# gabo99cas/minimal_volumetric_path_tracer

Hardware: AMD Instinct MI355X
Metric: Msamples/s (pixels×spp/s) at 1024²; per-channel RMSE vs CPU PPM (higher is better)
Workload: dtype f64; 1 GPU; ff 1024x1024x256spp default scene, sigma_a 0.001 sigma_s 0.009; width=1024, height=1024, spp=256, estimator=ff, parallelism=1 GPU, inflight=3

## Files before the change

minimal_volumetric_path_tracer_amd/_lib.py:

```python
from __future__ import annotations

import ctypes
import os
from ctypes import POINTER, c_char_p, c_double, c_int, c_int32, c_int64, c_uint64, c_void_p

import numpy as np

PKG_DIR = os.path.dirname(os.path.abspath(__file__))
LIB_PATH = os.environ.get("VPT_LIB") or os.path.join(PKG_DIR, "libvpt.so")
CLI_PATH = os.path.join(PKG_DIR, "vpt")

VPT_OK = 0
VPT_E_INVALID, VPT_E_TOO_MANY, VPT_E_NO_EMITTER, VPT_E_UNSUPPORTED, VPT_E_HIP, VPT_E_IO, VPT_E_INTERNAL = \
    -1, -2, -3, -4, -5, -6, -7
VPT_MAX_SPHERES = 64
FREE_FLIGHT, MIS_EQUIANGULAR, EXPLICIT_FREE, IMPLICIT_FREE, EXPLICIT_EQUIANGULAR, SURFACE_PT, RAY_MARCHING = 0, 1, 2, 3, 4, 5, 6
RAY_MARCHING_SA, RAY_MARCHING_GLOBAL, RAY_MARCHING_EXPLICIT = 7, 8, 9
HETERO_FREE = 10
HETERO_RATIO = 11
HETERO_EQUIANGULAR = 12
HETERO_MIS = 13
HETERO_CHROMATIC = 14
FB_F32, FB_F64 = 0, 1
GRID_NEAREST, GRID_TRILINEAR = 0, 1
# ... 138 lines not shown
                                        c_void_p, c_void_p, c_int, c_void_p, c_void_p, c_void_p, c_void_p, c_void_p, c_void_p,
                                        c_void_p, c_void_p, c_void_p]),
    ("vpt_grid_chroma_probe", c_int, [c_void_p, c_double, c_double, c_void_p, c_void_p, c_void_p, c_int, c_void_p, c_void_p,
                                      c_void_p, c_void_p, c_void_p, c_void_p]),
    ("vpt_grid_chroma_probe_host", c_int, [POINTER(vpt_grid_desc), c_void_p, c_int, c_int, c_void_p, c_void_p, c_void_p,
                                           c_void_p, c_void_p, c_int, c_void_p, c_void_p, c_void_p, c_void_p, c_void_p,
                                           c_void_p]),
    ("vpt_write_ppm", c_int, [c_char_p, c_void_p, c_int, c_int, c_int]),
    ("vpt_encode_ppm", c_int64, [c_void_p, c_int, c_int, c_int, c_void_p, c_int64]),
    ("vpt_last_error", c_char_p, []),
    ("vpt_abi_version", c_int, []),
    ("vpt_build_id", c_char_p, []),
]


def lib() -> ctypes.CDLL:
    global _lib
    if _lib is None:
        if not os.path.exists(LIB_PATH):
            raise RuntimeError(
                f"{LIB_PATH} is missing: build it with `python -c 'import __graft_entry__ as g; g.build()'` "
                "(or `make -C minimal_volumetric_path_tracer_amd/csrc`); there is no CPU fallback"
            )
        L = ctypes.CDLL(LIB_PATH)
        for name, res, args in PROTOTYPES:
            fn = getattr(L, name)
            fn.restype = res
            fn.argtypes = args
        _lib = L
    return _lib


def build_id() -> str:
    return lib().vpt_build_id().decode()


def check(rc: int) -> None:
    if rc != VPT_OK:
        msg = lib().vpt_last_error()
        raise VPTError(rc, msg.decode() if msg else "")
# ... 1 lines not shown
```

minimal_volumetric_path_tracer_amd/csrc/vpt_device.h:

```cpp
#ifndef VPT_DEVICE_H
#define VPT_DEVICE_H

#include <hip/hip_runtime.h>
#include <stdint.h>

#include <type_traits>

#include "vpt_math.h"
#include "vpt_rng.h"
#include "vpt_scene.h"

#define VPT_DEV __device__ static inline __attribute__((always_inline))
#define VPT_PI 3.14159265358979323846
#define VPT_MAXFLOAT ((double)3.40282346638528859812e+38F)
#define VPT_DBL_MAX 1.7976931348623157e+308
#ifndef VPT_ISECT_UNROLL
#define VPT_ISECT_UNROLL 5
#endif
#ifndef VPT_DECIDE_GROUP
#define VPT_DECIDE_GROUP 5
#endif
static_assert(VPT_DECIDE_GROUP >= 1, "spheres are taken G >= 1 at a time");

namespace vpt {

#define VPT_UNLIKELY(c) __builtin_expect(!!(c), 0)
#define VPT_LIKELY(c) __builtin_expect(!!(c), 1)

#define ISECT_SQRT(x) vm_sqrt(x)
#ifndef VPT_ISECT_CLASS
#define VPT_ISECT_CLASS 1
#endif

#ifndef VPT_SECTIONS
#define VPT_SECTIONS 0
#endif
enum {
    SECT_SCHED = 0, SECT_LOAD, SECT_S_PLIGHT, SECT_S_MIS, SECT_S_MIS_ISECT, SECT_S_BDSF, SECT_M_SS, SECT_M_SS_DIR,
    SECT_M_SS_ISECT, SECT_M_SS_SHADOW, SECT_M_PHASE, SECT_CONT, SECT_A_PREP, SECT_A_DECIDE, SECT_A_ISECT, SECT_STORE,
    SECT_S_TOTAL, SECT_M_TOTAL, SECT_A_CAMERA, SECT_A_DECIDE_IN, SECT_M_SHADOW_IN, SECT_A_CAMERA_IN, SECT_M_EQA,
    SECT_M_TR, SECT_A_UNIT, SECT_A_R2, SECT_A_PICK, SECT_A_LOG, SECT_A_CLASS, SECT_A_ALLFRESH, SECT_USED,
    SECT_N = 32
};
#if VPT_SECTIONS
static __device__ unsigned long long g_vpt_sect[3 * SECT_N];
__device__ static inline __attribute__((always_inline)) uint32_t* sect_lds()
{
    __shared__ uint32_t a[8][3 * SECT_USED];
    return &a[(threadIdx.x >> 6) & 7][0];
}
#endif
__device__ static inline __attribute__((always_inline)) uint32_t sect_now()
{
#if VPT_SECTIONS
    return (uint32_t)__builtin_amdgcn_s_memtime();
#else
// ... 3 lines not shown
__device__ static inline __attribute__((always_inline)) void sect_add(int k, uint32_t t0)
{
#if VPT_SECTIONS
    const uint32_t dt = sect_now() - t0;
    const unsigned long long act = (unsigned long long)__ballot(1);
    const int first = __ffsll(act) - 1;
    if ((int)(threadIdx.x & 63) == first) {
        uint32_t* a = sect_lds();
        a[k] += dt;
        a[SECT_USED + k] += 1;
        a[2 * SECT_USED + k] += (uint32_t)__popcll(act);
    }
#else
    (void)k;
    (void)t0;
#endif
}
__device__ static inline __attribute__((always_inline)) void sect_init()
{
#if VPT_SECTIONS
    for (int l = threadIdx.x & 63; l < 3 * SECT_USED; l += 64) sect_lds()[l] = 0;
#endif
}
__device__ static inline __attribute__((always_inline)) void sect_flush()
{
#if VPT_SECTIONS
    for (int l = threadIdx.x & 63; l < 3 * SECT_USED; l += 64) {
        const uint32_t v = sect_lds()[l];
        atomicAdd(&g_vpt_sect[l < SECT_USED ? l : l < 2 * SECT_USED ? SECT_N + l - SECT_USED : 2 * SECT_N + l - 2 * SECT_USED],
                  (unsigned long long)v);
// ... 144 lines not shown
        double cc = ocx * ocx + ocy * ocy + ocz * ocz;
        double det = b * b - cc + g.r2;
        sphere_test<ZR>(b, det, i, tmin, id, contact);
    }
    smp.tests(skip3 ? S->n_non3 : n);
    if (contact) {
        t = tmin;
        return 1;
    }
    t = 0;
    return 0;
}

template <int G, bool COUNT, bool ZR = false, class TAB = const double (*)[4]>
VPT_DEV int scene_intersect_grouped(const DevScene* __restrict__ S, Sampler<COUNT>& smp, dv3 o, dv3 d, double& t,
                                    int& id, bool cam = false, TAB cam_oc = nullptr)
{
    static_assert(G >= 1, "spheres are taken G >= 1 at a time");
    double tmin = VPT_DBL_MAX;
    contact_t contact = 0;
    const int n = S->n;
    int i = 0;
    for (; i + G <= n; i += G) {
        double b[G], det[G];
        if (cam) {
#pragma unroll
            for (int k = 0; k < G; ++k) {
                const double ocx = cam_oc[i + k][0], ocy = cam_oc[i + k][1], ocz = cam_oc[i + k][2], cc = cam_oc[i + k][3];
                b[k] = ocx * d.x + ocy * d.y + ocz * d.z;
                det[k] = b[k] * b[k] - cc + S->geo[i + k].r2;
            }
        } else {
#pragma unroll
            for (int k = 0; k < G; ++k) {
                const GeoSphere g = S->geo[i + k];
                const double ocx = o.x - g.px, ocy = o.y - g.py, ocz = o.z - g.pz;
                b[k] = ocx * d.x + ocy * d.y + ocz * d.z;
// ... 1171 lines not shown

template <bool COUNT>
VPT_DEV bool continue_path(Sampler<COUNT>& smp, const Path& p, const Medium& m)
{
    if (m.max_depth > 0 && p.depth >= m.max_depth) return false;
    if (COUNT) smp.cnt.iterations++;
    const double q = 1 - 0.6;
    return !(smp.next() < q);
}

template <int EST>
VPT_DEV constexpr bool est_free_flight() { return EST == 0 || EST == 2 || EST == 3; }

template <int EST, bool COUNT, bool HOIST = false, class TAB = const double (*)[4]>
VPT_DEV int decide(const DevScene* __restrict__ S, Sampler<COUNT>& smp, Path& p, Event& e, const Medium& m,
                   bool cam = false, TAB cam_oc = nullptr, uint64_t m_emitter = 0)
{
    constexpr bool hoist = HOIST && (EST == 0 || EST == 2);
    const double sigma_t = m.sigma_a + m.sigma_s;
    int id = 0;
    double t = 0.0;
    int h_count = 0, h_src = 0;
    double h_x = 0;
    gm_log_pair h_lp = {0, 0};
    if constexpr (hoist) {
        h_count = S->n_emit;
        if (VPT_LIKELY(h_count != 0)) {
            h_src = emit_pick(S, (int)(smp.next() * h_count), h_count);
            h_x = 1 - smp.next();
            h_lp = gm_log_pair_of(h_x);
        }
    }
    SECT_BEGIN(di);
#if VPT_DUP == DUP_DECIDE_ISECT
    {
        dv3 o2 = p.o, d2 = p.d;
        vpt_opaque(o2);
        vpt_opaque(d2);
        double t2 = 0;
        int id2 = 0;
        const int h2 = scene_intersect_grouped<VPT_DECIDE_GROUP>(S, smp, o2, d2, t2, id2);
        vpt_sink(t2);
        vpt_sink(id2);
        vpt_sink(h2);
    }
#endif
    const bool hit = scene_intersect_grouped<VPT_DECIDE_GROUP>(S, smp, p.o, p.d, t, id, cam, cam_oc);
    SECT_END(di, SECT_A_ISECT);
    if constexpr (EST == 5) {
        if (COUNT) smp.cnt.iterations++;
        e.t = t;
        e.id = id;
        e.src = 0;
        if (!hit) return EV_END;
        if (S->sph[id].radiance[0] > 0) {
            if (p.depth < 1) p.L = sph_rad(S, id);
            return EV_END;
        }
        return EV_SURF;
    }
    if (!hit) t = VPT_MAXFLOAT;
    e.t = t;
    e.id = id;
// ... 619 lines not shown
```

minimal_volumetric_path_tracer_amd/csrc/vpt_host.cpp:

```cpp
#include <math.h>
#include <stdarg.h>
#include <stdio.h>
#include <stdlib.h>
#include <string.h>

#include <string>
#include <vector>

#include <thread>

#include "vpt_accum.h"
#include "vpt_grid.h"
#include "vpt_grid_eqa.h"
#include "vpt_grid_mis.h"
#include "vpt_grid_chroma.h"
#include "vpt_internal.h"
#include "vpt_rng.h"

static thread_local std::string g_err;

int vpt_fail(int code, const char* fmt, ...)
{
    char buf[512];
    va_list ap;
    va_start(ap, fmt);
    vsnprintf(buf, sizeof buf, fmt, ap);
// ... 28 lines not shown
    }
    return VPT_OK;
}

void vpt_int_cam_table(const double* o, const double* centre, size_t stride, int n, double (*oc)[4])
{
    for (int i = 0; i < n; ++i, centre += stride) {
        const double ocx = o[0] - centre[0], ocy = o[1] - centre[1], ocz = o[2] - centre[2];
        oc[i][0] = ocx;
        oc[i][1] = ocy;
        oc[i][2] = ocz;
        oc[i][3] = ocx * ocx + ocy * ocy + ocz * ocz;
    }
}

extern "C" {

int vpt_debug_cam_table(const vpt_sphere* spheres, int n, const double* o, double* out)
{
    if (!spheres || !o || !out || n < 0 || n > VPT_MAX_SPHERES) return vpt_fail(VPT_E_INVALID, "vpt_debug_cam_table: bad arguments");
    vpt_int_cam_table(o, spheres[0].p, sizeof(vpt_sphere) / sizeof(double), n, (double (*)[4])out);
    return VPT_OK;
}

const char* vpt_last_error(void) { return g_err.c_str(); }
int vpt_abi_version(void) { return VPT_ABI_VERSION; }

uint64_t vpt_stream_state(uint64_t seed, uint64_t pixel_idx, uint64_t sample)
{
    return vpt_stream_start(seed, pixel_idx, sample);
}
// ... 444 lines not shown
```

minimal_volumetric_path_tracer_amd/csrc/vpt_internal.h:

```cpp
#ifndef VPT_INTERNAL_H
#define VPT_INTERNAL_H

#include <stddef.h>

#include "../../include/vpt.h"

int vpt_fail(int code, const char* fmt, ...);
void vpt_clear_error(void);

int vpt_int_device(const vpt_context* ctx);
const unsigned* vpt_int_guard_flag(const vpt_context* ctx);
int vpt_int_check_guard(vpt_context* ctx, const char* who);
int vpt_int_check_params(const vpt_context* ctx, const vpt_params* p);
int vpt_int_pool_pass(vpt_context* ctx, const vpt_params* p, int C, int k0, int k1, const unsigned* d_tiles,
                      unsigned n_tiles, double* d_partials, unsigned* d_queue);

void vpt_int_cam_table(const double* o, const double* centre, size_t stride, int n, double (*oc)[4]);

int vpt_int_grid_check(const vpt_grid_desc* desc, const float* density, const char* who);
int vpt_int_emission_check(const float* eps, size_t nv, const double rgb[3], const char* who);

#endif
```

minimal_volumetric_path_tracer_amd/csrc/vpt_kernels.hip:

```cpp
#include <hip/hip_runtime.h>

#include <math.h>
#include <stdlib.h>
#include <string.h>

#include <memory>
#include <mutex>
#include <vector>

#include "vpt_device.h"
#include "vpt_pool.h"
#include "vpt_wave.h"
#include "vpt_hetero_mis.h"
#include "vpt_hetero_chroma.h"
#include "vpt_hetero_launch.h"

#ifndef VPT_MIS_TU
#define VPT_MIS_TU 1
#endif
#if VPT_MIS_TU
namespace vpt {
extern template __global__ void pool_kernel<1, false>(PoolParams P0, Medium m0, const DevScene* __restrict__ S,
                                                      unsigned long long* counters, unsigned long long* stats);
extern template __global__ void pool_kernel<1, false, true>(PoolParams P0, Medium m0, const DevScene* __restrict__ S,
// ... 194 lines not shown
    const dv3 din = mk(dx, dy, dz);
    if (i < n) {
        Sampler<false> smp;
        smp.X = X[i];
        smp.g = g;
        smp.cnt.tests = smp.cnt.iterations = smp.cnt.draw_mismatch = 0;
        const dv3 w = phase_sample(smp, din);
        dirs[3 * i] = w.x;
        dirs[3 * i + 1] = w.y;
        dirs[3 * i + 2] = w.z;
        Xout[i] = smp.X;
    }
    if (i < nw) vals[i] = phase_value(g, din, mk(wl[3 * i], wl[3 * i + 1], wl[3 * i + 2]));
}

bool is_finite(double v) { return v == v && v - v == 0.0; }

unsigned long long* g_pool_stats = nullptr;

}

struct StreamSlot {
    hipStream_t stream;
    unsigned* d_queue;
    double* d_partials;
    size_t partials_bytes;
    hipEvent_t done;
    unsigned long long used;
};
constexpr int MAX_STREAM_SLOTS = 8;
constexpr int LAUNCH_LOG2_MAX = 26;

struct vpt_context {
    int device;
    DevScene* d_scene;
    DevScene h_scene;
    int has_scene;
    unsigned long long* d_counters;
    unsigned* d_guard;
    unsigned guard_bias = 0;
    std::mutex mu;
    std::vector<std::unique_ptr<StreamSlot>> slots;
    unsigned long long tick = 0;
    int launch_log2 = LAUNCH_LOG2_MAX;
    vpt_grid_view* d_grid = nullptr;
    float* d_rho = nullptr;
    int has_grid = 0;
    int maj_block = 0;
    float* d_maj = nullptr;
    vpt_grid_view h_grid = {};
    int grid_interp = 0;
    double* d_emit = nullptr;
    double mis_fraction = 0.5;
    double chroma_a[3] = {1.0, 1.0, 1.0}, chroma_s[3] = {1.0, 1.0, 1.0};
};

static int stream_slot(vpt_context* ctx, hipStream_t stream, size_t pbytes, StreamSlot** out)
{
    StreamSlot* sl = nullptr;
    for (auto& x : ctx->slots)
        if (x->stream == stream) sl = x.get();
    if (!sl && (int)ctx->slots.size() < MAX_STREAM_SLOTS) {
        std::unique_ptr<StreamSlot> n(new StreamSlot{stream, nullptr, nullptr, 0, nullptr, 0});
        HIP_OK(hipMalloc((void**)&n->d_queue, sizeof(unsigned)));
        const hipError_t e = hipEventCreateWithFlags(&n->done, hipEventDisableTiming);
        if (e != hipSuccess) {
            (void)hipFree(n->d_queue);
            return vpt_fail(VPT_E_HIP, "hipEventCreateWithFlags: %s", hipGetErrorString(e));
        }
// ... 14 lines not shown
    if (pbytes > sl->partials_bytes) {
        if (sl->d_partials) HIP_OK(hipFreeAsync(sl->d_partials, stream));
        sl->d_partials = nullptr;
        sl->partials_bytes = 0;
        HIP_OK(hipMallocAsync((void**)&sl->d_partials, pbytes, stream));
        sl->partials_bytes = pbytes;
    }
    sl->used = ++ctx->tick;
    *out = sl;
    return VPT_OK;
}

static int slot_done(StreamSlot* sl, hipStream_t stream)
{
    HIP_OK(hipEventRecord(sl->done, stream));
    return VPT_OK;
}

static int check_medium(const vpt_medium* m)
{
    if (!m) return vpt_fail(VPT_E_INVALID, "medium is NULL");
    if (!is_finite(m->sigma_a) || !is_finite(m->sigma_s) || m->sigma_a < 0 || m->sigma_s < 0)
        return vpt_fail(VPT_E_INVALID, "sigma_a/sigma_s must be finite and >= 0");
    if (!is_finite(m->hg_g) || m->hg_g <= -1.0 || m->hg_g >= 1.0) return vpt_fail(VPT_E_INVALID, "hg_g must be in (-1, 1)");
    if (m->max_depth < 0) return vpt_fail(VPT_E_INVALID, "max_depth must be >= 0");
    if (m->estimator < 0 || m->estimator >= VPT_NUM_ESTIMATORS)
        return vpt_fail(VPT_E_INVALID, "unknown estimator %d", m->estimator);
    return VPT_OK;
}

// ... 244 lines not shown
}

template <int EST>
static int pool_enqueue(vpt_context* ctx, const KParams& K, PoolParams& Q, uint64_t first, uint64_t units, double* partials,
                        unsigned* queue, hipStream_t stream)
{
    const DevScene* S = ctx->d_scene;
    constexpr bool COUNT = false;
    int blocks = 0;
    Q.partials = partials;
    Q.queue = queue;
    Q.guard = ctx->d_guard;
    Q.guard_bias = ctx->guard_bias;
    memset(Q.cam_oc, 0, sizeof Q.cam_oc);
    vpt_int_cam_table(K.o, &ctx->h_scene.geo[0].px, sizeof(GeoSphere) / sizeof(double), ctx->h_scene.n, Q.cam_oc);
    const Medium m = medium_of(K);
    constexpr bool HAS_TILES = EST <= 1;
    const bool tiles = Q.tile_map != nullptr;
    if (tiles && !HAS_TILES)
        return vpt_fail(VPT_E_UNSUPPORTED, "estimator %d renders whole tile sets only (tile subsets: estimators 0 and 1)", EST);
    int rc;
    if constexpr (HAS_TILES) {
        rc = tiles ? persistent_grid(ctx, pool_kernel<EST, COUNT, true>, &blocks, VPT_POOL_THREADS)
                   : persistent_grid(ctx, pool_kernel<EST, COUNT>, &blocks, VPT_POOL_THREADS);
    } else {
        rc = persistent_grid(ctx, pool_kernel<EST, COUNT>, &blocks, VPT_POOL_THREADS);
    }
    if (rc) return rc;
    const uint64_t need = (units + POOL - 1) / POOL;
    if ((uint64_t)blocks > need) blocks = (int)need;
// ... 9 lines not shown
        HIP_OK(hipMemsetAsync(g_pool_stats + TL0, 0xFF, 3 * TL_MAXWG * sizeof(unsigned long long), stream));
        stats = g_pool_stats;
    }
    for (uint64_t u0 = 0; u0 < units; u0 += max_units) {
        Q.unit0 = (unsigned)(first + u0);
        Q.nunits = (unsigned)(units - u0 < max_units ? units - u0 : max_units);
        HIP_OK(hipMemsetAsync(Q.queue, 0, sizeof(unsigned), stream));
        if constexpr (HAS_TILES) {
            if (tiles) pool_kernel<EST, COUNT, true><<<dim3((unsigned)blocks), dim3(VPT_POOL_THREADS), 0, stream>>>(Q, m, S, K.counters, stats);
            else pool_kernel<EST, COUNT><<<dim3((unsigned)blocks), dim3(VPT_POOL_THREADS), 0, stream>>>(Q, m, S, K.counters, stats);
        } else {
            pool_kernel<EST, COUNT><<<dim3((unsigned)blocks), dim3(VPT_POOL_THREADS), 0, stream>>>(Q, m, S, K.counters, stats);
        }
        HIP_OK(hipGetLastError());
    }
    return VPT_OK;
}

template <int EST, int FB>
static int launch_pool(vpt_context* ctx, KParams K, hipStream_t stream)
{
    [[maybe_unused]] constexpr bool COUNT = false;
    int rc;
    const bool wave = EST <= 1 && env_int("VPT_WAVE_KERNEL", 0);
    if (!wave) {
        PoolParams Q;
        uint64_t first = 0, units = 0;
        const vpt_chunk_layout lay = vpt_chunks(K.spp, K.chunk, K.taper);
        rc = pool_plan(K, lay, 0, lay.n, nullptr, (unsigned)K.tiles_x * (unsigned)K.tiles_y, Q, &first, &units);
        if (rc) return rc;
        const size_t pbytes = (size_t)K.shard_rows * (size_t)K.w * (size_t)Q.nch * 3 * sizeof(double);
// ... 137 lines not shown
}

void vpt_context_destroy(vpt_context* ctx)
{
    if (!ctx) return;
    int prev = 0;
    (void)hipGetDevice(&prev);
    (void)hipSetDevice(ctx->device);
    if (ctx->d_scene) (void)hipFree(ctx->d_scene);
    if (ctx->d_counters) (void)hipFree(ctx->d_counters);
    if (ctx->d_guard) (void)hipFree(ctx->d_guard);
    if (ctx->d_grid) (void)hipFree(ctx->d_grid);
    if (ctx->d_rho) (void)hipFree(ctx->d_rho);
    if (ctx->d_maj) (void)hipFree(ctx->d_maj);
    if (ctx->d_emit) (void)hipFree(ctx->d_emit);
    for (auto& sl : ctx->slots) {
        if (sl->done) (void)hipEventSynchronize(sl->done);
        if (sl->d_partials) (void)hipFree(sl->d_partials);
        if (sl->d_queue) (void)hipFree(sl->d_queue);
        if (sl->done) (void)hipEventDestroy(sl->done);
    }
    (void)hipSetDevice(prev);
    delete ctx;
}

int vpt_set_scene(vpt_context* ctx, const vpt_sphere* s, int n)
{
    vpt_clear_error();
    if (!ctx || !s) return vpt_fail(VPT_E_INVALID, "vpt_set_scene: NULL argument");
    if (n < 1) return vpt_fail(VPT_E_INVALID, "vpt_set_scene: empty scene");
// ... 27 lines not shown
        if (h.geo[i].skey & 1) h.m_skey1 |= bit;
        if (h.geo[i].skey & 2) h.m_skey2 |= bit;
        if (q.r > 0 && q.radiance[0] > 0) h.mis_light[h.n_mis++] = i;
        if (q.material == 3) h.n_mat3++;
    }
    h.n_non3 = n - h.n_mat3;
    vpt_erand48_jump(2 * h.n_mis + 5, &h.kp_sa, &h.kp_sc);
    h.emit_all_radiance = 1;
    for (int i = 0; i < n; ++i)
        if (!h.geo[i].emitter && (s[i].radiance[0] != 0 || s[i].radiance[1] != 0 || s[i].radiance[2] != 0))
            h.emit_all_radiance = 0;
    HIP_OK(hipSetDevice(ctx->device));
    HIP_OK(hipMemcpy(ctx->d_scene, &h, sizeof h, hipMemcpyHostToDevice));
    ctx->h_scene = h;
    ctx->has_scene = 1;
    return VPT_OK;
}

static hipError_t majorant_upload(vpt_grid_view* G, int B, const float* density, float** d_maj)
{
    int32_t nb[3];
    vpt_grid_majorant_counts(G->n, B, nb);
    std::vector<float> maj((size_t)nb[0] * (size_t)nb[1] * (size_t)nb[2]);
    if (G->interp) vpt_grid_majorant_build_tl(G->n, B, density, maj.data());
    else vpt_grid_majorant_build(G->n, B, density, maj.data());
    hipError_t e = hipMalloc((void**)d_maj, maj.size() * sizeof(float));
    if (e == hipSuccess) e = hipMemcpy(*d_maj, maj.data(), maj.size() * sizeof(float), hipMemcpyHostToDevice);
    if (e == hipSuccess) vpt_grid_view_set_majorant(G, B, *d_maj);
    return e;
}
// ... 705 lines not shown
    ctx->guard_bias = bias;
    if (bias == 0) HIP_OK(hipMemset(ctx->d_guard, 0, sizeof(unsigned)));
    return VPT_OK;
}
extern "C" int vpt_debug_kill_jump(vpt_context* ctx, int draws)
{
    vpt_clear_error();
    if (!ctx || !ctx->has_scene) return vpt_fail(VPT_E_INVALID, "NULL context or no scene");
    if (draws < 0) return vpt_fail(VPT_E_INVALID, "draws must be >= 0");
    DevScene& h = ctx->h_scene;
    vpt_erand48_jump(draws > 0 ? draws : 2 * h.n_mis + 5, &h.kp_sa, &h.kp_sc);
    HIP_OK(hipSetDevice(ctx->device));
    HIP_OK(hipMemcpy(ctx->d_scene, &h, sizeof h, hipMemcpyHostToDevice));
    return VPT_OK;
}
```

minimal_volumetric_path_tracer_amd/csrc/vpt_pool.h:

```cpp
#ifndef VPT_POOL_H
#define VPT_POOL_H

#include "vpt_chunks.h"
#include "vpt_device.h"

namespace vpt {

#ifndef VPT_POOL_DEBUG
#define VPT_POOL_DEBUG 0
#endif
#ifndef VPT_POOL_THREADS
#define VPT_POOL_THREADS 512
#endif
#ifndef VPT_POOL_WGS
#define VPT_POOL_WGS 1
#endif
#ifndef VPT_KILL_RINGS
#define VPT_KILL_RINGS 1
#endif
#ifndef VPT_SCHED_PRIO
#define VPT_SCHED_PRIO 3
#endif
#ifndef VPT_PREP_TRIES
#define VPT_PREP_TRIES 3
// ... 64 lines not shown
    int band_rows, band_stride, band_offset;
    int tiles_x, nch;
    vpt_chunk_layout lay;
    unsigned level_units;
    unsigned nunits;
    unsigned unit0;
    uint64_t seed;
    double o[3], d[3], cx[3], cy[3];
    int sh_lu, sh_tx, sh_br, sh_bs, sh_c;
    double rw, rh;
    double* partials;
    unsigned* queue;
    unsigned* guard;
    unsigned guard_bias;
    const unsigned* tile_map;
    double cam_oc[VPT_MAX_SPHERES][4];
};
static_assert(sizeof(PoolParams) + sizeof(Medium) + 3 * sizeof(void*) <= 4096, "pool_kernel's arguments: at most 4 KB");

#ifndef VPT_P_KARG
#define VPT_P_KARG 1
#endif
#if VPT_P_KARG && defined(__HIP_DEVICE_COMPILE__)
typedef const __attribute__((address_space(4))) PoolParams PoolParamsK;
__device__ __forceinline__ PoolParamsK& pool_params_at_use()
{
    uint64_t a = (uint64_t)(uintptr_t)__builtin_amdgcn_kernarg_segment_ptr();
    __asm__ volatile("" : "+s"(a));
    return *(PoolParamsK*)a;
}
// ... 173 lines not shown
    return VPT_KILL_RINGS && (EST == 0 || EST == 1 || EST == 2 || EST == 4);
}
__device__ __forceinline__ bool path_ends_after_event(uint64_t X, int depth, const Medium& m, uint64_t ja, uint64_t jc)
{
    if (m.max_depth > 0 && depth + 1 >= m.max_depth) return true;
    return vpt_erand48_value(vpt_erand48_skip(X, ja, jc)) < 1 - 0.6;
}

template <int EST, bool TMAP, bool COUNT>
__device__ __forceinline__ int stage_a(TaskPool& sh, const PoolParams& P0, const DevScene* __restrict__ S,
                                       const Medium& m, Sampler<COUNT>& smp, Task& t, bool active, int lane,
                                       uint64_t below, bool dbg, ADbg& D)
{
    VPT_PARAMS(P0);
    bool done = !active, parked = false, fresh = false;
    if (active && t.killed) {
        t.acc = add(t.p.L, t.acc);
        t.in_path = false;
        t.killed = false;
    }
    const unsigned long long c0 = dbg_clock(dbg);
    SECT_BEGIN(pr);
    int round = 0;
    uint32_t t_r2 = 0;
    while (true) {
        if (dbg) ++D.rounds;
        ++round;
        if (round == 2) t_r2 = sect_now();
        const bool need = !done && !parked && t.c1 == 0;
        const uint64_t needm = __ballot(need);
// ... 58 lines not shown
                ++t.i;
                if (dbg) ++D.samples;
                if (EST == 5) {
                    t.X = X0;
                    t.in_path = true;
                    fresh = true;
                } else {
                    if (COUNT) smp.cnt.iterations++;
                    if (!(vpt_erand48_value(vpt_erand48_skip3(X0)) < 1 - 0.6)) {
                        t.X = X0;
                        t.in_path = true;
                        fresh = true;
                    }
                }
            }
            if (VPT_UNLIKELY(!t.in_path && t.i == t.c1)) {
                store_partial(P0, t);
                t.c1 = 0;
            }
        }
        const uint64_t waiting = __ballot(!done && !parked && !t.in_path);
        if (waiting == 0) break;
        if ((VPT_PREP_ROUNDS > 0 && round >= VPT_PREP_ROUNDS) || __popcll(waiting) < VPT_PREP_MORE_MIN) {
            if (!done && !t.in_path) parked = true;
            break;
        }
    }
    if (round >= 2) sect_add(SECT_A_R2, t_r2);
    SECT_END(pr, SECT_A_PREP);
    SECT_BEGIN(cam);
// ... 14 lines not shown
            vpt_opaque(py);
            vpt_sink(pool_camera_dir(P0, jx2, jy2, px, py));
        }
#endif
        t.p.d = pool_camera_dir(P0, jx, jy, (int)(t.pix & 0xFFFFu), (int)(t.pix >> 16));
        t.p.beta = mk(1, 1, 1);
        t.p.L = mk(0, 0, 0);
        t.p.depth = 0;
        if (EST == 5) t.e.pdf = 1;
        t.X = smp.X;
        SECT_END(ci, SECT_A_CAMERA_IN);
    }
    SECT_END(cam, SECT_A_CAMERA);
    const unsigned long long c1 = dbg_clock(dbg);
    int result = parked ? R_A : R_DONE;
    SECT_BEGIN(dc);
    if (!done && !parked) {
        SECT_BEGIN(dci);
        smp.X = t.X;
#if VPT_DUP == DUP_DECIDE
        {
            Path p2 = t.p;
            Event e2 = t.e;
            vpt_opaque(p2);
            vpt_opaque(e2);
            Sampler<COUNT> s2 = smp;
            vpt_opaque(s2.X);
            vpt_sink(decide<EST>(S, s2, p2, e2, m));
            vpt_sink(p2);
            vpt_sink(e2);
            vpt_sink(s2.X);
        }
#endif
        constexpr bool CAM = kill_predicted_est<EST>() && !COUNT;
        const bool cam = CAM && __ballot(!fresh) == 0;
#if VPT_SECTIONS
        if (__ballot(!fresh) == 0) sect_add(SECT_A_ALLFRESH, sect_now());
#endif
        constexpr bool HOIST = EST == 0 || EST == 2;
        uint64_t w_emitter = 0, w_point = 0, w_skey1 = 0, w_skey2 = 0, w_kpa = 0, w_kpc = 0;
        if constexpr (HOIST) {
            w_emitter = S->m_emitter, w_point = S->m_point, w_skey1 = S->m_skey1, w_skey2 = S->m_skey2;
            w_kpa = S->kp_sa, w_kpc = S->kp_sc;
            __asm__ volatile("" : "+s"(w_emitter), "+s"(w_point), "+s"(w_skey1), "+s"(w_skey2), "+s"(w_kpa), "+s"(w_kpc));
        }
        const int ev = decide<EST, COUNT, true>(S, smp, t.p, t.e, m, cam, P.cam_oc, w_emitter);
        SECT_BEGIN(cl);
        t.X = smp.X;
        if (ev == EV_END) {
            t.acc = add(t.p.L, t.acc);
            t.in_path = false;
            result = R_A;
        } else if (ev == EV_SURF) {
            const int sk = sph_flag(HOIST ? w_skey1 : S->m_skey1, t.e.id) | (sph_flag(HOIST ? w_skey2 : S->m_skey2, t.e.id) << 1);
            result = R_S + (sk == 0 ? (EST == 3 || EST == 5 ? 0 : sph_flag(HOIST ? w_point : S->m_point, t.e.src)) : sk);
            if (kill_predicted_est<EST>() && !COUNT && sk == 0 &&
                path_ends_after_event(t.X, t.p.depth, m, HOIST ? w_kpa : S->kp_sa, HOIST ? w_kpc : S->kp_sc))
                result += R_SD - R_S;
        } else {
            result = R_M + (EST == 3 ? 0 : sph_flag(HOIST ? w_point : S->m_point, t.e.src));
            if (!(EST == 1 || EST == 4)) t.e.t = t.e.dist;
// ... 289 lines not shown
```

Baseline: 7389 Msamples/s.

## Precompute per-pixel conservative sphere-hit certificates to cull camera-ray intersection tests

Adds a kernel that, per pixel, conservatively bounds which spheres the camera ray footprint can hit first, using recursive subdivision of the pixel and interval bounds on the ray-sphere roots. The resulting 16-bit mask is cached per scene version, camera and resolution, and is read when a fresh path starts. The masks are OR-reduced across the wavefront with DPP, and when all lanes are fresh the camera intersection tests only the listed spheres. This aims to cut sphere tests on primary rays, at the cost of a one-time mask kernel, extra memory, event bookkeeping and a per-lane global load.

New measurement: 7411 Msamples/s, median of 6. No clear change (+0.3%).

```diff
diff --git a/minimal_volumetric_path_tracer_amd/_lib.py b/minimal_volumetric_path_tracer_amd/_lib.py
--- a/minimal_volumetric_path_tracer_amd/_lib.py
+++ b/minimal_volumetric_path_tracer_amd/_lib.py
@@ -176,6 +176,13 @@
 ]
 
 
+DEBUG_PROTOTYPES = [
+    ("vpt_debug_cam_cert", c_int, [c_void_p, c_int, c_void_p, c_void_p, c_void_p, c_void_p, c_int, c_int, c_void_p]),
+    ("vpt_debug_cam_cert_enable", c_int, [c_void_p, c_int]),
+    ("vpt_debug_cam_cert_read", c_int, [c_void_p, c_void_p, ctypes.c_size_t, POINTER(c_int), POINTER(c_int)]),
+]
+
+
 def lib() -> ctypes.CDLL:
     global _lib
     if _lib is None:
@@ -185,7 +192,7 @@
                 "(or `make -C minimal_volumetric_path_tracer_amd/csrc`); there is no CPU fallback"
             )
         L = ctypes.CDLL(LIB_PATH)
-        for name, res, args in PROTOTYPES:
+        for name, res, args in PROTOTYPES + DEBUG_PROTOTYPES:
             fn = getattr(L, name)
             fn.restype = res
             fn.argtypes = args
diff --git a/minimal_volumetric_path_tracer_amd/csrc/vpt_cam_cert.h b/minimal_volumetric_path_tracer_amd/csrc/vpt_cam_cert.h
--- /dev/null
+++ b/minimal_volumetric_path_tracer_amd/csrc/vpt_cam_cert.h
@@ -0,0 +1,134 @@
+#ifndef VPT_CAM_CERT_H
+#define VPT_CAM_CERT_H
+
+#include <stddef.h>
+#include <stdint.h>
+
+#ifdef __HIPCC__
+#define VPT_CC __host__ __device__ static inline __attribute__((always_inline))
+#else
+#define VPT_CC static inline
+#endif
+
+#define VPT_CERT_MAX_SPHERES 16
+#define VPT_CERT_LEVELS 6
+
+struct vpt_cert_in {
+    double d[3], cx[3], cy[3];
+    int w, h, n, pad_;
+    double oc[VPT_CERT_MAX_SPHERES][4];
+    double r2[VPT_CERT_MAX_SPHERES];
+};
+
+VPT_CC double vpt_cert_abs(double v) { return v < 0 ? -v : v; }
+VPT_CC int vpt_cert_finite(double v) { return v - v == 0.0; }
+
+VPT_CC uint32_t vpt_cert_cell_mask(const vpt_cert_in* c, int x, int y, double ox, double oy, double hs, uint32_t among)
+{
+    const int n = c->n;
+    const uint32_t full = among;
+    const double fx = ((double)x + ox) / c->w - .5, fy = ((double)y + oy) / c->h - .5;
+    const double vx = c->cx[0] * fx + c->cy[0] * fy + c->d[0];
+    const double vy = c->cx[1] * fx + c->cy[1] * fy + c->d[1];
+    const double vz = c->cx[2] * fx + c->cy[2] * fy + c->d[2];
+    const double sa = hs / c->w, sb = hs / c->h;
+    const double ax = c->cx[0] * sa, ay = c->cx[1] * sa, az = c->cx[2] * sa;
+    const double bx = c->cy[0] * sb, by = c->cy[1] * sb, bz = c->cy[2] * sb;
+    const double dv = __builtin_sqrt(ax * ax + ay * ay + az * az + bx * bx + by * by + bz * bz +
+                                     2 * vpt_cert_abs(ax * bx + ay * by + az * bz));
+    const double vn = __builtin_sqrt(vx * vx + vy * vy + vz * vz);
+    if (!(vn > 0) || !vpt_cert_finite(vn) || !vpt_cert_finite(dv)) return full;
+    const double ratio = dv / vn;
+    if (!(ratio < 0.1)) return full;
+    const double inv = 1.0 / vn;
+    const double ux = vx * inv, uy = vy * inv, uz = vz * inv;
+    double mag = 0;
+    for (int k = 0; k < 3; ++k) mag += vpt_cert_abs(c->cx[k]) + vpt_cert_abs(c->cy[k]) + vpt_cert_abs(c->d[k]);
+    const double sn = 1.01 * ratio, rnd = 1e-14 * (1 + mag * inv);
+    if (!vpt_cert_finite(rnd)) return full;
+
+    uint32_t keep = 0;
+    double lower[VPT_CERT_MAX_SPHERES];
+    double U = 1.7976931348623157e+308;
+    for (int i = 0; i < n; ++i) {
+        lower[i] = 0.0001;
+        if (!(among >> i & 1u)) continue;
+        const double cc = c->oc[i][3], r2 = c->r2[i];
+        const double noc = __builtin_sqrt(cc) * (1 + 1e-15), rr = __builtin_sqrt(r2);
+        const double bc = c->oc[i][0] * ux + c->oc[i][1] * uy + c->oc[i][2] * uz;
+        const double perp = __builtin_sqrt((cc - bc * bc > 0 ? cc - bc * bc : 0) + 1e-14 * cc);
+        const double beta = vpt_cert_abs(bc) * sn * sn + perp * sn + noc * (rnd + 2e-15);
+        const double bL = bc - beta, bH = bc + beta;
+        const double E = 4e-15 * (cc + r2), Et = 4e-15 * (noc + rr);
+        const double q = cc - r2;
+        if (!vpt_cert_finite(bL) || !vpt_cert_finite(bH) || !vpt_cert_finite(bL * bL) || !vpt_cert_finite(bH * bH) ||
+            !vpt_cert_finite(E) || !(Et <= 1e-5)) {
+            keep |= 1u << i;
+            continue;
+        }
+        if (q < -2 * E) {
+            const double hi = -bL + __builtin_sqrt(bL * bL - q + E) + Et;
+            const double lo = -bH + __builtin_sqrt(bH * bH - q - E) - Et;
+            if (hi <= 0.0001) continue;
+            keep |= 1u << i;
+            if (lo > 0.0001) {
+                lower[i] = lo;
+                U = hi < U ? hi : U;
+            }
+        } else if (q > 2 * E) {
+            if (bL >= 0) continue;
+            const double dH = bL * bL - q + E;
+            if (dH < 0) continue;
+            const double sH = __builtin_sqrt(dH);
+            if (-bL + sH + Et <= 0.0001) continue;
+            keep |= 1u << i;
+            const double lo = -bL - sH - Et;
+            if (lo > 0.0001) lower[i] = lo;
+            const double dL = bH * bH - q - E;
+            if (bH < 0 && dL > 0 && lo > 0.0001) {
+                const double hi = -bH - __builtin_sqrt(dL) + Et;
+                U = hi < U ? hi : U;
+            }
+        } else {
+            keep |= 1u << i;
+        }
+    }
+    for (int i = 0; i < n; ++i)
+        if (lower[i] > U) keep &= ~(1u << i);
+    return keep;
+}
+
+VPT_CC int vpt_cert_popcount(uint32_t m)
+{
+    int k = 0;
+    for (; m; m &= m - 1) ++k;
+    return k;
+}
+
+VPT_CC uint16_t vpt_cert_pixel_mask(const vpt_cert_in* c, int x, int y)
+{
+    const uint32_t m0 = vpt_cert_cell_mask(c, x, y, 0.0, 0.0, 0.5, (1u << c->n) - 1u);
+    if (vpt_cert_popcount(m0) <= 1) return (uint16_t)m0;
+    uint32_t cell[3 * VPT_CERT_LEVELS + 4], from[3 * VPT_CERT_LEVELS + 4];
+    int sp = 0;
+    for (int k = 0; k < 4; ++k) cell[sp] = 1u << 24 | (uint32_t)(k >> 1) << 12 | (uint32_t)(k & 1), from[sp++] = m0;
+    uint32_t m = 0;
+    while (sp > 0 && m != m0) {
+        const uint32_t e = cell[--sp], among = from[sp];
+        if ((among & ~m) == 0) continue;
+        const int level = (int)(e >> 24), j = (int)(e >> 12 & 0xFFFu), i = (int)(e & 0xFFFu);
+        const double hs = 0.5 / (double)(1 << level);
+        const uint32_t cm = vpt_cert_cell_mask(c, x, y, (2 * i + 1) * hs - 0.5, (2 * j + 1) * hs - 0.5, hs, among);
+        if (vpt_cert_popcount(cm) <= 1 || level == VPT_CERT_LEVELS) {
+            m |= cm;
+            continue;
+        }
+        for (int k = 0; k < 4; ++k)
+            cell[sp] = (uint32_t)(level + 1) << 24 | (uint32_t)(2 * j + (k >> 1)) << 12 | (uint32_t)(2 * i + (k & 1)), from[sp++] = cm;
+    }
+    return (uint16_t)m;
+}
+
+VPT_CC size_t vpt_cert_index(int w, int h, int x, int y) { return (size_t)(h - 1 - y) * (size_t)w + (size_t)x; }
+
+#endif
diff --git a/minimal_volumetric_path_tracer_amd/csrc/vpt_device.h b/minimal_volumetric_path_tracer_amd/csrc/vpt_device.h
--- a/minimal_volumetric_path_tracer_amd/csrc/vpt_device.h
+++ b/minimal_volumetric_path_tracer_amd/csrc/vpt_device.h
@@ -21,6 +21,10 @@
 #define VPT_DECIDE_GROUP 5
 #endif
 static_assert(VPT_DECIDE_GROUP >= 1, "spheres are taken G >= 1 at a time");
+#ifndef VPT_CERT_GROUP
+#define VPT_CERT_GROUP 4
+#endif
+static_assert(VPT_CERT_GROUP >= 1, "spheres are taken G >= 1 at a time");
 
 namespace vpt {
 
@@ -39,7 +43,7 @@
     SECT_SCHED = 0, SECT_LOAD, SECT_S_PLIGHT, SECT_S_MIS, SECT_S_MIS_ISECT, SECT_S_BDSF, SECT_M_SS, SECT_M_SS_DIR,
     SECT_M_SS_ISECT, SECT_M_SS_SHADOW, SECT_M_PHASE, SECT_CONT, SECT_A_PREP, SECT_A_DECIDE, SECT_A_ISECT, SECT_STORE,
     SECT_S_TOTAL, SECT_M_TOTAL, SECT_A_CAMERA, SECT_A_DECIDE_IN, SECT_M_SHADOW_IN, SECT_A_CAMERA_IN, SECT_M_EQA,
-    SECT_M_TR, SECT_A_UNIT, SECT_A_R2, SECT_A_PICK, SECT_A_LOG, SECT_A_CLASS, SECT_A_ALLFRESH, SECT_USED,
+    SECT_M_TR, SECT_A_UNIT, SECT_A_R2, SECT_A_PICK, SECT_A_LOG, SECT_A_CLASS, SECT_A_ALLFRESH, SECT_A_CAM_CAST, SECT_A_CERT_POP, SECT_USED,
     SECT_N = 32
 };
 #if VPT_SECTIONS
@@ -73,6 +77,21 @@
 #else
     (void)k;
     (void)t0;
+#endif
+}
+__device__ static inline __attribute__((always_inline)) void sect_count(int k, uint32_t v)
+{
+#if VPT_SECTIONS
+    const unsigned long long act = (unsigned long long)__ballot(1);
+    if ((int)(threadIdx.x & 63) == __ffsll(act) - 1) {
+        uint32_t* a = sect_lds();
+        a[k] += v;
+        a[SECT_USED + k] += 1;
+        a[2 * SECT_USED + k] += (uint32_t)__popcll(act);
+    }
+#else
+    (void)k;
+    (void)v;
 #endif
 }
 __device__ static inline __attribute__((always_inline)) void sect_init()
@@ -247,13 +266,37 @@
 
 template <int G, bool COUNT, bool ZR = false, class TAB = const double (*)[4]>
 VPT_DEV int scene_intersect_grouped(const DevScene* __restrict__ S, Sampler<COUNT>& smp, dv3 o, dv3 d, double& t,
-                                    int& id, bool cam = false, TAB cam_oc = nullptr)
+                                    int& id, bool cam = false, TAB cam_oc = nullptr, uint32_t cert = 0)
 {
     static_assert(G >= 1, "spheres are taken G >= 1 at a time");
     double tmin = VPT_DBL_MAX;
     contact_t contact = 0;
     const int n = S->n;
     int i = 0;
+    if (cert != 0) {
+        uint32_t rem = cert;
+        do {
+            int j[VPT_CERT_GROUP];
+            bool have[VPT_CERT_GROUP];
+            double b[VPT_CERT_GROUP], det[VPT_CERT_GROUP];
+#pragma unroll
+            for (int k = 0; k < VPT_CERT_GROUP; ++k) {
+                have[k] = rem != 0;
+                j[k] = have[k] ? __builtin_ctz(rem) : j[k > 0 ? k - 1 : 0];
+                rem &= rem - 1;
+            }
+#pragma unroll
+            for (int k = 0; k < VPT_CERT_GROUP; ++k) {
+                const double ocx = cam_oc[j[k]][0], ocy = cam_oc[j[k]][1], ocz = cam_oc[j[k]][2], cc = cam_oc[j[k]][3];
+                b[k] = ocx * d.x + ocy * d.y + ocz * d.z;
+                det[k] = b[k] * b[k] - cc + S->geo[j[k]].r2;
+            }
+#pragma unroll
+            for (int k = 0; k < VPT_CERT_GROUP; ++k)
+                if (have[k]) sphere_test<ZR>(b[k], det[k], j[k], tmin, id, contact);
+        } while (rem != 0);
+        i = n;
+    }
     for (; i + G <= n; i += G) {
         double b[G], det[G];
         if (cam) {
@@ -1455,7 +1498,7 @@
 
 template <int EST, bool COUNT, bool HOIST = false, class TAB = const double (*)[4]>
 VPT_DEV int decide(const DevScene* __restrict__ S, Sampler<COUNT>& smp, Path& p, Event& e, const Medium& m,
-                   bool cam = false, TAB cam_oc = nullptr, uint64_t m_emitter = 0)
+                   bool cam = false, TAB cam_oc = nullptr, uint64_t m_emitter = 0, uint32_t cert = 0)
 {
     constexpr bool hoist = HOIST && (EST == 0 || EST == 2);
     const double sigma_t = m.sigma_a + m.sigma_s;
@@ -1486,8 +1529,11 @@
         vpt_sink(h2);
     }
 #endif
-    const bool hit = scene_intersect_grouped<VPT_DECIDE_GROUP>(S, smp, p.o, p.d, t, id, cam, cam_oc);
+    const bool hit = scene_intersect_grouped<VPT_DECIDE_GROUP>(S, smp, p.o, p.d, t, id, cam, cam_oc, cert);
     SECT_END(di, SECT_A_ISECT);
+#if VPT_SECTIONS
+    if (cam) SECT_END(di, SECT_A_CAM_CAST);
+#endif
     if constexpr (EST == 5) {
         if (COUNT) smp.cnt.iterations++;
         e.t = t;
diff --git a/minimal_volumetric_path_tracer_amd/csrc/vpt_host.cpp b/minimal_volumetric_path_tracer_amd/csrc/vpt_host.cpp
--- a/minimal_volumetric_path_tracer_amd/csrc/vpt_host.cpp
+++ b/minimal_volumetric_path_tracer_amd/csrc/vpt_host.cpp
@@ -10,6 +10,7 @@
 #include <thread>
 
 #include "vpt_accum.h"
+#include "vpt_cam_cert.h"
 #include "vpt_grid.h"
 #include "vpt_grid_eqa.h"
 #include "vpt_grid_mis.h"
@@ -68,7 +69,44 @@
     }
 }
 
+bool vpt_int_cam_cert_in(const double* d, const double* cx, const double* cy, int w, int h, const double (*oc)[4],
+                         const double* r2, size_t stride, int n, vpt_cert_in* in)
+{
+    if (n < 1 || n > VPT_CERT_MAX_SPHERES) return false;
+    memset(in, 0, sizeof *in);
+    for (int k = 0; k < 3; ++k) {
+        in->d[k] = d[k];
+        in->cx[k] = cx[k];
+        in->cy[k] = cy[k];
+    }
+    in->w = w;
+    in->h = h;
+    in->n = n;
+    for (int i = 0; i < n; ++i, r2 += stride) {
+        for (int k = 0; k < 4; ++k) in->oc[i][k] = oc[i][k];
+        in->r2[i] = *r2;
+    }
+    return true;
+}
+
 extern "C" {
+
+int vpt_debug_cam_cert(const vpt_sphere* spheres, int n, const double* o, const double* d, const double* cx,
+                       const double* cy, int w, int h, uint16_t* out)
+{
+    if (!spheres || !o || !d || !cx || !cy || !out || n < 1 || n > VPT_MAX_SPHERES || w < 1 || h < 1 || w > 65535 || h > 65535)
+        return vpt_fail(VPT_E_INVALID, "vpt_debug_cam_cert: bad arguments");
+    if (n > VPT_CERT_MAX_SPHERES)
+        return vpt_fail(VPT_E_UNSUPPORTED, "vpt_debug_cam_cert: %d spheres > %d, the certificate is off", n, VPT_CERT_MAX_SPHERES);
+    double oc[VPT_CERT_MAX_SPHERES][4], r2[VPT_CERT_MAX_SPHERES];
+    vpt_int_cam_table(o, spheres[0].p, sizeof(vpt_sphere) / sizeof(double), n, oc);
+    for (int i = 0; i < n; ++i) r2[i] = spheres[i].r * spheres[i].r;
+    vpt_cert_in in;
+    vpt_int_cam_cert_in(d, cx, cy, w, h, oc, r2, 1, n, &in);
+    for (int y = 0; y < h; ++y)
+        for (int x = 0; x < w; ++x) out[vpt_cert_index(w, h, x, y)] = vpt_cert_pixel_mask(&in, x, y);
+    return VPT_OK;
+}
 
 int vpt_debug_cam_table(const vpt_sphere* spheres, int n, const double* o, double* out)
 {
diff --git a/minimal_volumetric_path_tracer_amd/csrc/vpt_internal.h b/minimal_volumetric_path_tracer_amd/csrc/vpt_internal.h
--- a/minimal_volumetric_path_tracer_amd/csrc/vpt_internal.h
+++ b/minimal_volumetric_path_tracer_amd/csrc/vpt_internal.h
@@ -17,6 +17,10 @@
 
 void vpt_int_cam_table(const double* o, const double* centre, size_t stride, int n, double (*oc)[4]);
 
+struct vpt_cert_in;
+bool vpt_int_cam_cert_in(const double* d, const double* cx, const double* cy, int w, int h, const double (*oc)[4],
+                         const double* r2, size_t stride, int n, struct vpt_cert_in* in);
+
 int vpt_int_grid_check(const vpt_grid_desc* desc, const float* density, const char* who);
 int vpt_int_emission_check(const float* eps, size_t nv, const double rgb[3], const char* who);
 
diff --git a/minimal_volumetric_path_tracer_amd/csrc/vpt_kernels.hip b/minimal_volumetric_path_tracer_amd/csrc/vpt_kernels.hip
--- a/minimal_volumetric_path_tracer_amd/csrc/vpt_kernels.hip
+++ b/minimal_volumetric_path_tracer_amd/csrc/vpt_kernels.hip
@@ -8,6 +8,7 @@
 #include <mutex>
 #include <vector>
 
+#include "vpt_cam_cert.h"
 #include "vpt_device.h"
 #include "vpt_pool.h"
 #include "vpt_wave.h"
@@ -232,6 +233,14 @@
     if (i < nw) vals[i] = phase_value(g, din, mk(wl[3 * i], wl[3 * i + 1], wl[3 * i + 2]));
 }
 
+__global__ __launch_bounds__(256) void cam_cert_kernel(vpt_cert_in in, uint16_t* out)
+{
+    const size_t p = (size_t)blockIdx.x * 256 + threadIdx.x;
+    if (p >= (size_t)in.w * (size_t)in.h) return;
+    const int fr = (int)(p / (size_t)in.w), x = (int)(p - (size_t)fr * (size_t)in.w);
+    out[p] = vpt_cert_pixel_mask(&in, x, in.h - 1 - fr);
+}
+
 bool is_finite(double v) { return v == v && v - v == 0.0; }
 
 unsigned long long* g_pool_stats = nullptr;
@@ -247,6 +256,23 @@
     unsigned long long used;
 };
 constexpr int MAX_STREAM_SLOTS = 8;
+
+struct CertUse {
+    hipStream_t stream;
+    hipEvent_t done;
+};
+struct CertEntry {
+    unsigned long long scene_version = 0;
+    double cam[12] = {};
+    int w = 0, h = 0;
+    uint16_t* d_mask = nullptr;
+    size_t bytes = 0;
+    hipEvent_t ready = nullptr;
+    std::vector<CertUse> uses;
+    unsigned long long used = 0;
+};
+constexpr int MAX_CERT_ENTRIES = 4;
+constexpr size_t CERT_MAX_BYTES = (size_t)64 << 20;
 constexpr int LAUNCH_LOG2_MAX = 26;
 
 struct vpt_context {
@@ -271,6 +297,11 @@
     double* d_emit = nullptr;
     double mis_fraction = 0.5;
     double chroma_a[3] = {1.0, 1.0, 1.0}, chroma_s[3] = {1.0, 1.0, 1.0};
+    std::mutex cert_mu;
+    std::vector<std::unique_ptr<CertEntry>> certs;
+    unsigned long long scene_version = 0, cert_tick = 0;
+    int cert_off = 0;
+    CertEntry* cert_last = nullptr;
 };
 
 static int stream_slot(vpt_context* ctx, hipStream_t stream, size_t pbytes, StreamSlot** out)
@@ -315,6 +346,79 @@
 static int slot_done(StreamSlot* sl, hipStream_t stream)
 {
     HIP_OK(hipEventRecord(sl->done, stream));
+    return VPT_OK;
+}
+
+static int cam_cert(vpt_context* ctx, bool est_casts_from_table, const KParams& K, const PoolParams& Q, hipStream_t stream,
+                    CertEntry** out)
+{
+    *out = nullptr;
+    const size_t bytes = (size_t)K.w * (size_t)K.h * sizeof(uint16_t);
+    std::lock_guard<std::mutex> lock(ctx->cert_mu);
+    ctx->cert_last = nullptr;
+    if (!est_casts_from_table || ctx->cert_off || ctx->h_scene.n > VPT_CERT_MAX_SPHERES || bytes > CERT_MAX_BYTES)
+        return VPT_OK;
+    double cam[12];
+    for (int i = 0; i < 3; ++i) cam[i] = K.o[i], cam[3 + i] = K.d[i], cam[6 + i] = K.cx[i], cam[9 + i] = K.cy[i];
+    CertEntry* e = nullptr;
+    for (auto& x : ctx->certs)
+        if (x->scene_version == ctx->scene_version && x->w == K.w && x->h == K.h && memcmp(x->cam, cam, sizeof cam) == 0)
+            e = x.get();
+    if (e) {
+        HIP_OK(hipStreamWaitEvent(stream, e->ready, 0));
+    } else {
+        if ((int)ctx->certs.size() < MAX_CERT_ENTRIES) {
+            std::unique_ptr<CertEntry> n(new CertEntry());
+            HIP_OK(hipEventCreateWithFlags(&n->ready, hipEventDisableTiming));
+            ctx->certs.push_back(std::move(n));
+            e = ctx->certs.back().get();
+        } else {
+            for (auto& x : ctx->certs)
+                if (!e || x->used < e->used) e = x.get();
+            HIP_OK(hipStreamWaitEvent(stream, e->ready, 0));
+            for (const CertUse& u : e->uses) HIP_OK(hipStreamWaitEvent(stream, u.done, 0));
+        }
+        e->w = e->h = 0;
+        if (bytes > e->bytes) {
+            if (e->d_mask) HIP_OK(hipFreeAsync(e->d_mask, stream));
+            e->d_mask = nullptr;
+            e->bytes = 0;
+            HIP_OK(hipMallocAsync((void**)&e->d_mask, bytes, stream));
+            e->bytes = bytes;
+        }
+        vpt_cert_in in;
+        if (!vpt_int_cam_cert_in(K.d, K.cx, K.cy, K.w, K.h, Q.cam_oc, &ctx->h_scene.geo[0].r2, sizeof(GeoSphere) / sizeof(double),
+                                 ctx->h_scene.n, &in))
+            return VPT_OK;
+        const size_t npix = (size_t)K.w * (size_t)K.h;
+        cam_cert_kernel<<<dim3((unsigned)((npix + 255) / 256)), dim3(256), 0, stream>>>(in, e->d_mask);
+        HIP_OK(hipGetLastError());
+        HIP_OK(hipEventRecord(e->ready, stream));
+        e->scene_version = ctx->scene_version;
+        memcpy(e->cam, cam, sizeof cam);
+        e->w = K.w;
+        e->h = K.h;
+    }
+    e->used = ++ctx->cert_tick;
+    ctx->cert_last = e;
+    *out = e;
+    return VPT_OK;
+}
+
+static int cam_cert_done(vpt_context* ctx, CertEntry* e, hipStream_t stream)
+{
+    if (!e) return VPT_OK;
+    std::lock_guard<std::mutex> lock(ctx->cert_mu);
+    CertUse* u = nullptr;
+    for (CertUse& x : e->uses)
+        if (x.stream == stream) u = &x;
+    if (!u) {
+        CertUse n{stream, nullptr};
+        HIP_OK(hipEventCreateWithFlags(&n.done, hipEventDisableTiming));
+        e->uses.push_back(n);
+        u = &e->uses.back();
+    }
+    HIP_OK(hipEventRecord(u->done, stream));
     return VPT_OK;
 }
 
@@ -589,6 +693,11 @@
     Q.guard_bias = ctx->guard_bias;
     memset(Q.cam_oc, 0, sizeof Q.cam_oc);
     vpt_int_cam_table(K.o, &ctx->h_scene.geo[0].px, sizeof(GeoSphere) / sizeof(double), ctx->h_scene.n, Q.cam_oc);
+    CertEntry* cert = nullptr;
+    constexpr bool CASTS_FROM_TABLE = VPT_KILL_RINGS && (EST == 0 || EST == 1 || EST == 2 || EST == 4);
+    const int rcc = cam_cert(ctx, CASTS_FROM_TABLE, K, Q, stream, &cert);
+    if (rcc) return rcc;
+    Q.cert = cert ? cert->d_mask : nullptr;
     const Medium m = medium_of(K);
     constexpr bool HAS_TILES = EST <= 1;
     const bool tiles = Q.tile_map != nullptr;
@@ -628,7 +737,7 @@
         }
         HIP_OK(hipGetLastError());
     }
-    return VPT_OK;
+    return cam_cert_done(ctx, cert, stream);
 }
 
 template <int EST, int FB>
@@ -796,6 +905,15 @@
     if (ctx->d_rho) (void)hipFree(ctx->d_rho);
     if (ctx->d_maj) (void)hipFree(ctx->d_maj);
     if (ctx->d_emit) (void)hipFree(ctx->d_emit);
+    for (auto& e : ctx->certs) {
+        if (e->ready) (void)hipEventSynchronize(e->ready);
+        for (CertUse& u : e->uses) {
+            (void)hipEventSynchronize(u.done);
+            (void)hipEventDestroy(u.done);
+        }
+        if (e->d_mask) (void)hipFree(e->d_mask);
+        if (e->ready) (void)hipEventDestroy(e->ready);
+    }
     for (auto& sl : ctx->slots) {
         if (sl->done) (void)hipEventSynchronize(sl->done);
         if (sl->d_partials) (void)hipFree(sl->d_partials);
@@ -853,6 +971,7 @@
     HIP_OK(hipMemcpy(ctx->d_scene, &h, sizeof h, hipMemcpyHostToDevice));
     ctx->h_scene = h;
     ctx->has_scene = 1;
+    ++ctx->scene_version;
     return VPT_OK;
 }
 
@@ -1588,3 +1707,28 @@
     HIP_OK(hipMemcpy(ctx->d_scene, &h, sizeof h, hipMemcpyHostToDevice));
     return VPT_OK;
 }
+
+extern "C" int vpt_debug_cam_cert_enable(vpt_context* ctx, int on)
+{
+    vpt_clear_error();
+    if (!ctx) return vpt_fail(VPT_E_INVALID, "NULL context");
+    std::lock_guard<std::mutex> lock(ctx->cert_mu);
+    ctx->cert_off = on == 0;
+    return VPT_OK;
+}
+extern "C" int vpt_debug_cam_cert_read(vpt_context* ctx, uint16_t* out, size_t cap, int* w, int* h)
+{
+    vpt_clear_error();
+    if (!ctx || !out || !w || !h) return vpt_fail(VPT_E_INVALID, "vpt_debug_cam_cert_read: bad arguments");
+    HIP_OK(hipSetDevice(ctx->device));
+    HIP_OK(hipDeviceSynchronize());
+    std::lock_guard<std::mutex> lock(ctx->cert_mu);
+    const CertEntry* e = ctx->cert_last;
+    if (!e || !e->d_mask) return vpt_fail(VPT_E_INVALID, "vpt_debug_cam_cert_read: the last launch had no certificate");
+    const size_t npix = (size_t)e->w * (size_t)e->h;
+    if (npix > cap) return vpt_fail(VPT_E_INVALID, "vpt_debug_cam_cert_read: %zu masks > %zu", npix, cap);
+    HIP_OK(hipMemcpy(out, e->d_mask, npix * sizeof(uint16_t), hipMemcpyDeviceToHost));
+    *w = e->w;
+    *h = e->h;
+    return VPT_OK;
+}
diff --git a/minimal_volumetric_path_tracer_amd/csrc/vpt_pool.h b/minimal_volumetric_path_tracer_amd/csrc/vpt_pool.h
--- a/minimal_volumetric_path_tracer_amd/csrc/vpt_pool.h
+++ b/minimal_volumetric_path_tracer_amd/csrc/vpt_pool.h
@@ -102,6 +102,7 @@
     unsigned* guard;
     unsigned guard_bias;
     const unsigned* tile_map;
+    const uint16_t* cert;
     double cam_oc[VPT_MAX_SPHERES][4];
 };
 static_assert(sizeof(PoolParams) + sizeof(Medium) + 3 * sizeof(void*) <= 4096, "pool_kernel's arguments: at most 4 KB");
@@ -305,6 +306,9 @@
 {
     VPT_PARAMS(P0);
     bool done = !active, parked = false, fresh = false;
+    constexpr bool CERT = kill_predicted_est<EST>() && !COUNT;
+    uint32_t cmask = 0;
+    bool cert_asked = false;
     if (active && t.killed) {
         t.acc = add(t.p.L, t.acc);
         t.in_path = false;
@@ -393,6 +397,14 @@
                     }
                 }
             }
+            if constexpr (CERT) {
+                const uint16_t* cert = P.cert;
+                const int cw = P.w, ch = P.h;
+                if (cert != nullptr && fresh && !cert_asked) {
+                    cert_asked = true;
+                    cmask = cert[(size_t)(ch - 1 - (int)(t.pix >> 16)) * (size_t)cw + (size_t)(t.pix & 0xFFFFu)];
+                }
+            }
             if (VPT_UNLIKELY(!t.in_path && t.i == t.c1)) {
                 store_partial(P0, t);
                 t.c1 = 0;
@@ -437,6 +449,19 @@
     SECT_END(cam, SECT_A_CAMERA);
     const unsigned long long c1 = dbg_clock(dbg);
     int result = parked ? R_A : R_DONE;
+    uint32_t cert_or = 0;
+    if constexpr (CERT) {
+        if (__ballot(!done && !parked && !fresh) == 0) {
+            int v = (int)cmask;
+            v |= __builtin_amdgcn_update_dpp(0, v, 0x111, 0xF, 0xF, false);
+            v |= __builtin_amdgcn_update_dpp(0, v, 0x112, 0xF, 0xF, false);
+            v |= __builtin_amdgcn_update_dpp(0, v, 0x114, 0xF, 0xF, false);
+            v |= __builtin_amdgcn_update_dpp(0, v, 0x118, 0xF, 0xF, false);
+            v |= __builtin_amdgcn_update_dpp(0, v, 0x142, 0xA, 0xF, false);
+            v |= __builtin_amdgcn_update_dpp(0, v, 0x143, 0xC, 0xF, false);
+            cert_or = (uint32_t)__builtin_amdgcn_readlane(v, 63);
+        }
+    }
     SECT_BEGIN(dc);
     if (!done && !parked) {
         SECT_BEGIN(dci);
@@ -460,6 +485,9 @@
 #if VPT_SECTIONS
         if (__ballot(!fresh) == 0) sect_add(SECT_A_ALLFRESH, sect_now());
 #endif
+#if VPT_SECTIONS
+        if (CERT && cam) sect_count(SECT_A_CERT_POP, (uint32_t)__popc(cert_or ? cert_or : (1u << S->n) - 1u));
+#endif
         constexpr bool HOIST = EST == 0 || EST == 2;
         uint64_t w_emitter = 0, w_point = 0, w_skey1 = 0, w_skey2 = 0, w_kpa = 0, w_kpc = 0;
         if constexpr (HOIST) {
@@ -467,7 +495,7 @@
             w_kpa = S->kp_sa, w_kpc = S->kp_sc;
             __asm__ volatile("" : "+s"(w_emitter), "+s"(w_point), "+s"(w_skey1), "+s"(w_skey2), "+s"(w_kpa), "+s"(w_kpc));
         }
-        const int ev = decide<EST, COUNT, true>(S, smp, t.p, t.e, m, cam, P.cam_oc, w_emitter);
+        const int ev = decide<EST, COUNT, true>(S, smp, t.p, t.e, m, cam, P.cam_oc, w_emitter, cam ? cert_or : 0u);
         SECT_BEGIN(cl);
         t.X = smp.X;
         if (ev == EV_END) {
```
